# truemeat001/Simple-Raytracing-Render

Measured on AMD Instinct MI355X. Metric: Msamples/s (rays x bounces) + HBM GB/s vs roofline, Cornell+teapot 1024spp, higher is better.
Workload: dtype f32

## Files before the change

### include/srr_capi.h

```cpp
#ifndef SRR_CAPI_H
#define SRR_CAPI_H

#include <stddef.h>
#include <stdint.h>

#ifdef __cplusplus
extern "C" {
#endif

#define SRR_OK 0
#define SRR_EINVAL (-22)
#define SRR_ENOMEM (-12)
#define SRR_ENODEV (-19)
#define SRR_ENOTSUP (-95)
#define SRR_EIO (-5)

typedef struct srr_scene srr_scene;
typedef struct srr_renderer srr_renderer;

const char* srr_last_error(void);
const char* srr_version(void);

srr_scene* srr_scene_create(void);
void srr_scene_destroy(srr_scene* s);
int srr_scene_from_text(const char* text, srr_scene** out);
int srr_scene_text_handle(const srr_scene* s, int text_id);
int srr_scene_set_lcg(srr_scene* s, uint64_t state);
#define SRR_DIGEST_PARTS 21
int srr_scene_digest(const srr_scene* s, uint64_t* out, uint64_t* parts);
uint64_t srr_scene_get_lcg(const srr_scene* s);
double srr_scene_drand48(srr_scene* s);

int srr_constant_texture(srr_scene* s, float r, float g, float b);
int srr_image_texture(srr_scene* s, const unsigned char* rgb, int nx, int ny);
int srr_image_texture_file(srr_scene* s, const char* path);
int srr_image_texture_gen(srr_scene* s, int nx, int ny, uint32_t seed, int kind);
int srr_checker_texture(srr_scene* s, int even_tex, int odd_tex);
int srr_noise_texture(srr_scene* s, float scale);

int srr_lambertian(srr_scene* s, int albedo_tex);
int srr_orennayar(srr_scene* s, int albedo_tex, float sigma_deg);
int srr_beckmann(srr_scene* s, int albedo_tex, float roughx, float roughy);
int srr_metal(srr_scene* s, float r, float g, float b, float fuzz);
int srr_dielectric(srr_scene* s, float ref_idx);
int srr_diffuse_light(srr_scene* s, int emit_tex);
int srr_isotropic(srr_scene* s, int albedo_tex);

int srr_sphere(srr_scene* s, const float center[3], float radius, int mat);
int srr_moving_sphere(srr_scene* s, const float c0[3], const float c1[3], float t0, float t1, float radius,
                      int mat);
int srr_xy_rect(srr_scene* s, float x0, float x1, float y0, float y1, float k, int mat);
int srr_xz_rect(srr_scene* s, float x0, float x1, float z0, float z1, float k, int mat);
int srr_yz_rect(srr_scene* s, float y0, float y1, float z0, float z1, float k, int mat);
int srr_box(srr_scene* s, const float p0[3], const float p1[3], int mat);
int srr_triangle(srr_scene* s, const float p[9], int mat, const float* uv9, const float* n9);
int srr_flip_normals(srr_scene* s, int child);
int srr_translate(srr_scene* s, int child, const float offset[3]);
int srr_rotate_y(srr_scene* s, int child, float angle_deg);
int srr_rotate_x(srr_scene* s, int child, float angle_deg);
int srr_constant_medium(srr_scene* s, int boundary, float density, int tex);
int srr_hitable_list(srr_scene* s, const int* children, int n);
int srr_bvh_node(srr_scene* s, const int* children, int n, float time0, float time1);
// ... 110 lines not shown
```

### simple-raytracing-render_amd/csrc/capi.cpp

```cpp
#include <hip/hip_runtime.h>

#include <algorithm>
#include <chrono>
#include <cstdint>
#include <cstdio>
#include <cstring>
#include <map>
#include <memory>
#include <string>
#include <vector>

#include "../../include/srr_capi.h"
#include "imageio.h"
#include "meshio.h"
#include "../../include/srr/merl.h"
#include "multi.h"
#include "renderer.h"

using namespace srr;

struct srr_scene {
  Scene s;
};

// ... 74 lines not shown
  auto vec = [&blob](const auto& v) { blob(v.data(), v.size() * sizeof(v[0])); };
  vec(f.objs);
  blob(&f.n_world, sizeof f.n_world);
  vec(f.xforms);
  vec(f.spheres);
  vec(f.rects);
  vec(f.stris);
  vec(f.meshes);
  vec(f.nodes);
  vec(f.node4);
  vec(f.tri_pos);
  vec(f.tri_shade);
  vec(f.media);
  {
    std::vector<uint8_t> b;
    auto put = [&b](const void* p, size_t n) { b.insert(b.end(), (const uint8_t*)p, (const uint8_t*)p + n); };
    put(f.obvhs.data(), f.obvhs.size() * sizeof(DObvh));
    put(f.sgroups.data(), f.sgroups.size() * sizeof(DSGroup));
    put(f.sg_items.data(), f.sg_items.size() * sizeof(DSGItem));
    vec(b);
  }
  vec(f.obvh_children);
  vec(f.mats);
  vec(f.texs);
  vec(f.images);
  vec(f.perlin_ranvec);
  vec(f.perlin_perm);
  vec(f.lights);
  blob(&f.cam, sizeof f.cam);
  *out = h;
  return 0;
}

int srr_scene_set_lcg(srr_scene* s, uint64_t state) {
  if (!s) return fail(SRR_EINVAL, "null scene");
  s->s.lcg = state & 0xFFFFFFFFFFFFULL;
  return 0;
}
uint64_t srr_scene_get_lcg(const srr_scene* s) { return s ? s->s.lcg : 0; }
double srr_scene_drand48(srr_scene* s) { return s ? s->s.drand48() : 0.0; }

#define SCN(s) \
  if (!(s)) return fail(SRR_EINVAL, "null scene");
#define TEXOK(s, t) \
  if (!(s)->s.valid_tex(t)) return fail(SRR_EINVAL, "bad texture handle " + std::to_string(t));
#define MATOK(s, m) \
  if (!(s)->s.valid_mat(m)) return fail(SRR_EINVAL, "bad material handle " + std::to_string(m));
#define OBJOK(s, o) \
  if (!(s)->s.valid_obj(o)) return fail(SRR_EINVAL, "bad hitable handle " + std::to_string(o));

int srr_constant_texture(srr_scene* s, float r, float g, float b) {
  SCN(s);
  HTex t;
  t.kind = TEX_CONST;
  t.c[0] = r; t.c[1] = g; t.c[2] = b;
  return s->s.add_tex(std::move(t));
}
int srr_image_texture(srr_scene* s, const unsigned char* rgb, int nx, int ny) {
  SCN(s);
  if (!rgb || nx <= 0 || ny <= 0) return fail(SRR_EINVAL, "bad image");
  HTex t;
  t.kind = TEX_IMAGE;
  t.nx = nx;
  t.ny = ny;
  t.px.assign(rgb, rgb + (size_t)nx * ny * 3);
  return s->s.add_tex(std::move(t));
// ... 765 lines not shown
```

### simple-raytracing-render_amd/csrc/device_scene.h

```cpp
#pragma once
#include <cstdint>

namespace srr {

enum ObjKind : int32_t {
  OBJ_SPHERE = 0,
  OBJ_MSPHERE = 1,
  OBJ_RECT = 2,
  OBJ_TRI = 3,
  OBJ_MESH = 4,
  OBJ_MEDIUM = 5,
  OBJ_OBVH = 6,
  OBJ_SGROUP = 7,
};

enum XformKind : int32_t { XF_FLIP = 0, XF_TRANSLATE = 1, XF_ROTY = 2, XF_ROTX = 3 };

struct DXform {
  int32_t kind;
  float a, b, c;
};

constexpr int32_t kXfFlipBit = 1 << 30;
constexpr int32_t kXfCountMask = 0xFFFF;
// ... 2 lines not shown
  int32_t kind;
  int32_t xf_begin, xf_count;
  int32_t idx;
};

struct DSphere {
  float c0[3], c1[3];
  float t0, t1, r;
  int32_t mat;
};

struct DRect {
  int32_t kax, a0, a1, mat;
  float lo0, hi0, lo1, hi1, k;
  float pad[3];
};

struct TriShade {
  float n[9];
  float uv[6];
  int32_t mat;
};

constexpr int kNode4qWords = 16;

struct DMesh {
  int32_t node_off;
  int32_t tri_off;
  int32_t n_nodes, n_tris;
  int32_t node4_off;
  int32_t n_node4;
};

struct DObvh {
  int32_t node_off, n_nodes;
  int32_t child_off, n_children;
};

struct DObvhChild {
  int32_t obj_begin, obj_count;
};

constexpr int kSGroupMinRun = 8;

struct DSGroup {
  int32_t node_off, n_nodes;
  int32_t item_off, n_items;
};

struct DSGItem {
  DSphere s;
  int32_t pos;
  int32_t moving;
  int32_t obj;
  int32_t pad;
};

struct DMedium {
  int32_t bnd_begin, bnd_count;
  float density;
  int32_t phase_mat;
};

enum MatKind : int32_t {
  MAT_LAMBERTIAN = 0,
  MAT_ORENNAYAR = 1,
  MAT_BECKMANN = 2,
  MAT_METAL = 3,
  MAT_DIELECTRIC = 4,
  MAT_DIFFUSE_LIGHT = 5,
  MAT_ISOTROPIC = 6,
  MAT_COUNT = 7,
};

struct DMat {
  int32_t kind;
  int32_t tex;
  float p[4];
};

enum TexKind : int32_t { TEX_CONST = 0, TEX_IMAGE = 1, TEX_CHECKER = 2, TEX_NOISE = 3 };

struct DTex {
  int32_t kind;
  int32_t nx, ny;
  int32_t even, odd;
  int64_t off;
  float c[3];
};

enum LightKind : int32_t { LIGHT_NONE = 0, LIGHT_XZRECT = 1, LIGHT_SPHERE = 2, LIGHT_TRI = 3 };

struct DLight {
  int32_t kind;
// ... 15 lines not shown
```

### simple-raytracing-render_amd/csrc/kernels.h

```cpp
#pragma once
#include <hip/hip_runtime.h>

#include <cstdint>

#include "device_scene.h"

namespace srr {

struct SceneView {
  const DObj* objs;
  int n_world;
  int has_media;
  const DXform* xforms;
  const DSphere* spheres;
  const DRect* rects;
  const DStandaloneTri* stris;
  const DMesh* meshes;
  const float4* nodes;
  const float4* node4;
  int node4_lds;
  int node4_total;
  const float4* node4q;
  int node4_lds_q;
  int use_q;
  int quad_trace;
  int quad_max;
  int mesh_obj;
  const float4* tri_pos;
  const float4* tri_edge;
  const TriShade* tri_shade;
  const DMedium* media;
  const DObvh* obvhs;
  const DObvhChild* obvh_children;
  const DSGroup* sgroups;
  const DSGItem* sg_items;
  const DMat* mats;
  const DTex* texs;
  const uint8_t* images;
  const float* perlin_ranvec;
  const int32_t* perlin_perm;
  const DLight* lights;
  int n_lights;
  float light_weight;
  const DCamera* cam;
  const uint4* world_blob;
  int world_words;
  int world_off[10];
};

struct PathState {
  float4* ray_o;
  float4* ray_d;
  uint64_t* lcg;
  uint64_t* pcg;
  int32_t* depth;
  uint64_t* spec;
  int4* hit_w;
  float4* hit_p;
  float4* hit_n;
  float4* rec_a;
  float* sample;
  float* raw;
  uint8_t* rays;
};

struct BatchInfo {
  int32_t* active;
  int32_t* count;
  int act0;
  int slot0;
  const int32_t* pixels;
  const double* sobol;
  int p0;
  int n_paths;
  int s0, spp_batch;
  int s_base;
  int nx, ny;
  uint64_t base_seed;
};

// ... 97 lines not shown
```

### simple-raytracing-render_amd/csrc/kernels.hip

```cpp
#include <hip/hip_runtime.h>

#include <cfloat>
#include <algorithm>
#include <cstdint>
#include <cstdlib>
#include <cstring>

#include "device_scene.h"
#include "devmath.h"
#include "kernels.h"
#include "../../include/srr/merl.h"

namespace srr {
namespace dev {

SRR_D V3 sphere_center(const DSphere& s, float tm, bool moving) {
  V3 c0 = v3(s.c0[0], s.c0[1], s.c0[2]);
  if (!moving) return c0;
  V3 c1 = v3(s.c1[0], s.c1[1], s.c1[2]);
  return c0 + ((tm - s.t0) / (s.t1 - s.t0)) * (c1 - c0);
}

SRR_D bool sphere_hit(const DSphere& s, bool moving, const Ray& r, float tmin, float tmax, float& t) {
  V3 oc = r.o - sphere_center(s, r.tm, moving);
  float a = dot(r.d, r.d);
  float b = dot(oc, r.d);
  float c = dot(oc, oc) - s.r * s.r;
  float disc = b * b - a * c;
  if (disc > 0) {
    float sq = rsqrt_exact(disc);
    float temp = (-b - sq) / a;
    if (temp < tmax && temp > tmin) { t = temp; return true; }
    temp = (-b + sq) / a;
    if (temp < tmax && temp > tmin) { t = temp; return true; }
  }
  return false;
}

template <int KAX>
SRR_D bool rect_hit_t(const DRect& q, const Ray& r, float tmin, float tmax, float& t) {
  constexpr int A0 = KAX == 0 ? 1 : 0, A1 = KAX == 2 ? 1 : 2;
  const float tt = (q.k - r.o[KAX]) / r.d[KAX];
  if (tt < tmin || tt > tmax) return false;
  const float x = r.o[A0] + tt * r.d[A0];
  const float y = r.o[A1] + tt * r.d[A1];
  if (x < q.lo0 || x > q.hi0 || y < q.lo1 || y > q.hi1) return false;
  t = tt;
  return true;
}

#ifndef SRR_RECTAX
#define SRR_RECTAX 1
#endif
SRR_D bool rect_hit(const DRect& q, const Ray& r, float tmin, float tmax, float& t, float& u, float& v) {
#ifdef SRR_EXP_FASTRECT
  float tt = (q.k - r.o[q.kax]) * __builtin_amdgcn_rcpf(r.d[q.kax]);
#else
  float tt = (q.k - r.o[q.kax]) / r.d[q.kax];
#endif
  if (tt < tmin || tt > tmax) return false;
  float x = r.o[q.a0] + tt * r.d[q.a0];
  float y = r.o[q.a1] + tt * r.d[q.a1];
  if (x < q.lo0 || x > q.hi0 || y < q.lo1 || y > q.hi1) return false;
  u = (x - q.lo0) / (q.hi0 - q.lo0);
  v = (y - q.lo1) / (q.hi1 - q.lo1);
  t = tt;
  return true;
}

SRR_D bool tri_hit(V3 p0, V3 p1, V3 p2, bool front, V3 o, V3 dir, float& t, float& u, float& v) {
  V3 e1, e2;
  if (front) { e1 = p1 - p0; e2 = p2 - p0; }
  else { e1 = p0 - p1; e2 = p2 - p1; }
// ... 1149 lines not shown
      for (int i = first; i < first + count; ++i) {
        const DSGItem it = S.sg_items[i];
        const V3 oc = r.o - sphere_center(it.s, r.tm, it.moving != 0);
        const float a = dot(r.d, r.d);
        const float b = dot(oc, r.d);
        const float c = dot(oc, oc) - it.s.r * it.s.r;
        const float disc = b * b - a * c;
        if (!(disc > 0)) continue;
        const float sq = rsqrt_exact(disc);
        const float t1 = (-b - sq) / a;
        float v;
        if (t1 > tmin) v = t1;
        else {
          const float t2 = (-b + sq) / a;
          if (!(t2 > tmin)) continue;
          v = t2;
        }
        if (!(v < tmax)) continue;
        if (!found || v < best || (v == best && it.pos < best_pos)) {
          found = true;
          best = v;
          best_pos = it.pos;
          best_item = i;
        }
      }
    }
    node = (hit && leaf < 0) ? node + 1 : skip;
  }
  out_t = best;
  out_item = best_item;
  return found;
}

template <int TR, bool U = false>
SRR_D bool basic_hit(const SceneView& S, const DObj& ob, const Ray& lr, float tmin, float tmax, bool is_medium,
                     ObjHit& h, const TraceCtx& cx) {
  switch (ob.kind) {
    case OBJ_MESH: {
#ifdef SRR_EXP_NOMESH
      return false;
#endif
      MeshHit mh;
      const DMesh m = maybe_uni<U>(wload<TR>(S.meshes, ob.idx));
      bool hit;
      if (tr_mode(TR) == TR_BVH2) hit = mesh_hit<false>(S, m, lr, tmin, tmax, is_medium, mh, cx.ctr);
      else if (TR & TR_QUAD)
        hit = mesh_hit4_quad<tr_mode(TR) != TR_BVH4, tr_stride(TR)>(S, m, lr, tmin, tmax, is_medium, mh, cx);
      else if (TR & TR_Q)
        hit = mesh_hit4<tr_mode(TR) != TR_BVH4, false, true, tr_stride(TR)>(S, m, lr, tmin, tmax, is_medium, mh, cx);
      else
        hit = mesh_hit4<tr_mode(TR) != TR_BVH4, tr_mode(TR) == TR_BVH4_TIMED, false, tr_stride(TR), (TR & TR_SUSP) != 0>(
            S, m, lr, tmin, tmax, is_medium, mh, cx);
      if (!hit) return false;
      h.t = mh.t;
      h.prim = mh.tri;
      return true;
    }
    case OBJ_OBVH:
      return obvh_hit<TR>(S, S.obvhs[ob.idx], lr, tmin, tmax, is_medium, h.t, h.prim);
    case OBJ_SGROUP:
      return sgroup_hit<TR>(S, S.sgroups[ob.idx], lr, tmin, tmax, h.t, h.prim);
    case OBJ_MEDIUM:
      return false;
    default:
      return prim_hit<TR, U>(S, ob, lr, tmin, tmax, is_medium, h.t);
  }
}

template <int TR>
SRR_D bool list_hit(const SceneView& S, int b, int n, const Ray& r, float tmin, float tmax, float& t,
                    const TraceCtx& cx) {
  bool any = false;
  float closest = tmax;
  for (int k = 0; k < n; ++k) {
    const DObj ob = maybe_uni<SRR_UNIFORM != 0>(wload<TR>(S.objs, b + k));
    const Ray lr = chain_in<TR, SRR_UNIFORM != 0>(S, ob, r);
    float th = 0;
    bool hit;
    if (ob.kind == OBJ_MESH) {
      MeshHit mh;
      hit = mesh_hit<false>(S, wload<TR>(S.meshes, ob.idx), lr, tmin, closest, true, mh, nullptr);
      th = mh.t;
    } else if (ob.kind == OBJ_OBVH) {
      int po;
      hit = obvh_hit<TR>(S, S.obvhs[ob.idx], lr, tmin, closest, true, th, po);
    } else if (ob.kind == OBJ_MEDIUM) {
      hit = false;
    } else {
      hit = prim_hit<TR, SRR_UNIFORM != 0>(S, ob, lr, tmin, closest, true, th);
    }
    if (hit) {
      any = true;
      closest = th;
      t = th;
    }
  }
  return any;
}
// ... 44 lines not shown
    if (MEDIA && ob.kind == OBJ_MEDIUM) {
      hit = medium_hit<TR>(S, maybe_uni<SRR_UNIFORM != 0>(wload<TR>(S.media, ob.idx)), lr, tmin, closest, rng, h.t, cx);
      h.prim = -1;
    } else {
      hit = basic_hit<TR, SRR_UNIFORM != 0>(S, ob, lr, tmin, closest, false, h, cx);
    }
    if (hit) {
      closest = h.t;
      w.obj = k;
      w.prim = h.prim;
      w.t = h.t;
    }
  }
}

template <bool MEDIA, int TR>
SRR_D WorldHit world_hit(const SceneView& S, const Ray& r, Rng& rng, const TraceCtx& cx) {
  WorldHit w{-1, -1, 0};
  float closest = FLT_MAX;
  const float tmin = 0.001f;
  constexpr bool SUSP = (TR & TR_SUSP) != 0;
  const bool skip = MEDIA || S.mesh_obj < 0;
  int k_res = -1;
  if constexpr (SUSP) {
    if (skip && cx.resume) {
      const float4 v = *walk_save(cx, 2);
      k_res = __float_as_int(v.x);
      closest = v.y;
      w.obj = __float_as_int(v.z);
      w.prim = __float_as_int(v.w);
      w.t = closest;
    }
  }
  for (int k = 0; k < S.n_world; ++k) {
    const DObj ob = maybe_uni<SRR_UNIFORM != 0>(wload<TR>(S.objs, k));
    if constexpr (SUSP) {
      if (skip && (cx.susp || k < k_res)) continue;
      cx.obj_k = k;
    }
    Ray lr = chain_in<TR, SRR_UNIFORM != 0>(S, ob, r);
    ObjHit h;
    bool hit;
    if (MEDIA && ob.kind == OBJ_MEDIUM) {
      hit = medium_hit<TR>(S, maybe_uni<SRR_UNIFORM != 0>(wload<TR>(S.media, ob.idx)), lr, tmin, closest, rng, h.t, cx);
      h.prim = -1;
    } else {
      hit = basic_hit<TR, SRR_UNIFORM != 0>(S, ob, lr, tmin, closest, false, h, cx);
    }
    if (SUSP && skip && cx.susp) {
      *walk_save(cx, 2) = make_float4(__int_as_float(k), closest, __int_as_float(w.obj), __int_as_float(w.prim));
      continue;
    }
    if (hit) {
      closest = h.t;
      w.obj = k;
      w.prim = h.prim;
      w.t = h.t;
    }
  }
  return w;
}

struct HitRec {
  V3 p, n;
  float u, v;
  int mat;
};

#if SRR_XFAX
template <int KAX>
SRR_D void rect_rec(const DRect& q, const Ray& r, HitRec& h) {
  constexpr int A0 = KAX == 0 ? 1 : 0, A1 = KAX == 2 ? 1 : 2;
  const float tt = (q.k - r.o[KAX]) / r.d[KAX];
  const float x = r.o[A0] + tt * r.d[A0];
  const float y = r.o[A1] + tt * r.d[A1];
  h.u = (x - q.lo0) / (q.hi0 - q.lo0);
  h.v = (y - q.lo1) / (q.hi1 - q.lo1);
  h.n = v3(0.f);
  h.n.set(KAX, 1.f);
}
#endif

SRR_D void sphere_uv(V3 p, float& u, float& v) {
  float phi = ratan2(p.z, p.x);
  float theta = rasin(p.y);
  u = 1 - (phi + kPi) / (2 * kPi);
  v = (theta + kPi / 2) / kPi;
}

template <int TR = 0>
SRR_D void prim_record(const SceneView& S, const DObj& ob, const Ray& lr, float t, int prim, HitRec& h) {
  switch (ob.kind) {
    case OBJ_SPHERE:
    case OBJ_MSPHERE: {
      const DSphere& s = S.spheres[ob.idx];
      V3 c = sphere_center(s, lr.tm, ob.kind == OBJ_MSPHERE);
      h.p = lr.at(t);
      if (ob.kind == OBJ_SPHERE) sphere_uv((h.p - c) / s.r, h.u, h.v);
      h.n = (h.p - c) / s.r;
      h.mat = s.mat;
      break;
    }
    case OBJ_RECT: {
      const DRect& q = S.rects[ob.idx];
#if SRR_XFAX
      switch (q.kax) {
        case 0: rect_rec<0>(q, lr, h); break;
        case 1: rect_rec<1>(q, lr, h); break;
        default: rect_rec<2>(q, lr, h); break;
      }
#else
      float tt;
      rect_hit(q, lr, -FLT_MAX, FLT_MAX, tt, h.u, h.v);
      h.n = v3(0.f);
      h.n.set(q.kax, 1.f);
#endif
      h.p = lr.at(t);
      h.mat = q.mat;
      break;
    }
    case OBJ_TRI:
    case OBJ_MESH: {
      V3 p0, p1, p2;
      TriShade shv;
      if (ob.kind == OBJ_TRI) {
        DStandaloneTri T;
        if constexpr ((TR & TR_WL) != 0) {
          static_assert(sizeof(DStandaloneTri) == 25 * 4, "DStandaloneTri: 25 words");
          const __attribute__((address_space(3))) float* q =
              (const __attribute__((address_space(3))) float*)(S.stris + ob.idx);
          float* t = (float*)&T;
#pragma unroll
          for (int k = 0; k < 25; ++k) t[k] = q[k];
        } else {
          T = S.stris[ob.idx];
// ... 7 lines not shown
        float4 a = tp[0], b = tp[1], c = tp[2];
        p0 = v3(a.x, a.y, a.z);
        p1 = v3(b.x, b.y, b.z);
        p2 = v3(c.x, c.y, c.z);
        shv = S.tri_shade[prim];
      }
      const TriShade* sh = &shv;
      V3 dir = lr.d / length(lr.d);
      float tt, u, v;
      tri_hit(p0, p1, p2, true, lr.o, dir, tt, u, v);
      float a0 = 1 - u - v;
      float uvx = a0 * sh->uv[0] + u * sh->uv[2] + v * sh->uv[4];
      float uvy = a0 * sh->uv[1] + u * sh->uv[3] + v * sh->uv[5];
      h.u = uvx;
      h.v = uvy;
      V3 n0 = v3(sh->n[0], sh->n[1], sh->n[2]), n1 = v3(sh->n[3], sh->n[4], sh->n[5]),
         n2 = v3(sh->n[6], sh->n[7], sh->n[8]);
      h.n = unit_vector(a0 * n0 + u * n1 + v * n2);
      h.p = a0 * p0 + u * p1 + v * p2;
      h.mat = sh->mat;
      break;
    }
    case OBJ_MEDIUM: {
      h.p = lr.at(t);
      h.n = v3(1, 0, 0);
      h.mat = S.media[ob.idx].phase_mat;
      break;
    }
  }
}

template <int TR = 0>
SRR_D HitRec world_record(const SceneView& S, const Ray& r, const WorldHit& w) {
  const DObj& ob = S.objs[w.obj];
  Ray lr = chain_in<TR>(S, ob, r);
  HitRec h;
  h.u = 0;
  h.v = 0;
  if (ob.kind == OBJ_OBVH || ob.kind == OBJ_SGROUP) {
    const DObj& in = S.objs[ob.kind == OBJ_SGROUP ? S.sg_items[w.prim].obj : w.prim];
    prim_record<TR>(S, in, chain_in<TR>(S, in, lr), w.t, -1, h);
    chain_out(S, in, h.p, h.n);
  } else {
    prim_record<TR>(S, ob, lr, w.t, w.prim, h);
  }
  chain_out(S, ob, h.p, h.n);
  return h;
}

enum Family : int { FAM_TERM = 0, FAM_DIFF = 1, FAM_BECK = 2, FAM_SPEC = 3 };

SRR_D int family_of(int mat, int kind, int depth, int max_depth) {
  if (mat < 0 || kind == MAT_DIFFUSE_LIGHT || depth >= max_depth) return FAM_TERM;
  if (kind == MAT_LAMBERTIAN || kind == MAT_ORENNAYAR) return FAM_DIFF;
  if (kind == MAT_BECKMANN) return FAM_BECK;
  return FAM_SPEC;
}

SRR_D int hit_material(const SceneView& S, const WorldHit& w) {
  DObj ob = S.objs[w.obj];
  if (ob.kind == OBJ_OBVH) ob = S.objs[w.prim];
  else if (ob.kind == OBJ_SGROUP) ob = S.objs[S.sg_items[w.prim].obj];
  switch (ob.kind) {
    case OBJ_SPHERE:
    case OBJ_MSPHERE: return S.spheres[ob.idx].mat;
    case OBJ_RECT: return S.rects[ob.idx].mat;
    case OBJ_TRI: return S.stris[ob.idx].sh.mat;
    case OBJ_MESH: return S.tri_shade[w.prim].mat;
    case OBJ_MEDIUM: return S.media[ob.idx].phase_mat;
  }
  return -1;
}

SRR_D void store_hit(const SceneView& S, const PathState& P, int p, const WorldHit& w, int max_depth, int& fam) {
  if (w.obj < 0) {
// ... 1248 lines not shown
SRR_D const PathsArgs* paths_args() { return nullptr; }
#endif

template <bool MEDIA, bool ALLFAM, int MINB, bool TIMED = false, bool WL = true, bool QUAD = false, bool CQ = false,
          int BS = kPathsBlock, bool SP = false>
#ifdef SRR_NUM_VGPR
#define SRR_PATHS_VGPR_ATTR __attribute__((amdgpu_num_vgpr(SRR_NUM_VGPR)))
#else
#define SRR_PATHS_VGPR_ATTR
#endif
__global__ void __launch_bounds__(BS, MINB) SRR_PATHS_VGPR_ATTR k_paths(PathsArgs A) {
  static_assert(BS == kPathsBlock || BS == 1024, "block size");
  (void)A;
  uint64_t tp[8] = {0, 0, 0, 0, 0, 0, 0, 0};
  uint64_t tf[20] = {0, 0, 0, 0, 0, 0, 0, 0, 0, 0, 0, 0, 0, 0, 0, 0, 0, 0, 0, 0};
  uint64_t it = 0;
  constexpr int TR = TR_BVH4_PRUNE | (WL ? TR_WL : 0) | (QUAD ? TR_QUAD : 0) | (CQ ? TR_Q : 0) | (BS == 1024 ? TR_BIG : 0) |
                     ((SP && !QUAD && !CQ) ? TR_SUSP : 0);
  __shared__ uint4 s_world[WL ? kWorldLdsBytes / 16 : 1];
  const auto view = [&]() {
    SceneView S = paths_args()->S;
    if constexpr (WL) {
      const char* b = (const char*)s_world;
      S.objs = (const DObj*)(b + S.world_off[0]);
      S.xforms = (const DXform*)(b + S.world_off[1]);
      S.spheres = (const DSphere*)(b + S.world_off[2]);
      S.rects = (const DRect*)(b + S.world_off[3]);
      S.stris = (const DStandaloneTri*)(b + S.world_off[4]);
      S.meshes = (const DMesh*)(b + S.world_off[5]);
      S.media = (const DMedium*)(b + S.world_off[6]);
      S.mats = (const DMat*)(b + S.world_off[7]);
      S.texs = (const DTex*)(b + S.world_off[8]);
      S.lights = (const DLight*)(b + S.world_off[9]);
    }
    return S;
  };
  const auto work = []() { return PathWork(paths_args()->W); };
  __shared__ int s_node[kStack * BS];
  __shared__ float s_t[kStack * BS];
  constexpr bool RING = SRR_RAYRING && !QUAD;
  constexpr int kNodesLds = BS == 1024 ? kPathsLdsNodesBig : ((WL && RING) ? kPathsLdsNodesSmall : kPathsLdsNodes);
  __shared__ float4 s_n4[kNodesLds * 8];
  __shared__ float s_ring[RING ? kRingWords * BS : 1];
  const lds_ptr<float> ringw = to_lds(s_ring + (RING ? (threadIdx.x & ~63u) : 0));
  uint32_t ring_base = 0;
  const uint32_t n_paths = (uint32_t)paths_args()->W.n_paths;
  const uint64_t t_start = paths_args()->W.wave_times ? __builtin_amdgcn_s_memrealtime() : 0;
  {
    const SceneView S0 = paths_args()->S;
    if constexpr (WL)
      for (int i = threadIdx.x; i < S0.world_words; i += blockDim.x) s_world[i] = S0.world_blob[i];
    const int n_lds_nodes = CQ ? min(S0.node4_total, 2 * kNodesLds) : min(S0.node4_total, kNodesLds);
    if (CQ)
      for (int i = threadIdx.x; i < n_lds_nodes * 4; i += blockDim.x) s_n4[i] = S0.node4q[i];
    else
      for (int i = threadIdx.x; i < n_lds_nodes * 8; i += blockDim.x) s_n4[i] = S0.node4[i];
  }
  __syncthreads();
  const int slot = blockIdx.x * blockDim.x + threadIdx.x;
  const auto rec_at = [&](const PathWork& W, int k) -> float4* {
    int s = slot;
    asm volatile("" : "+v"(s));
    return W.rec + ((size_t)k * W.lanes + s);
  };
  int g = -1;
  uint32_t pool = 0, pool_end = 0;
// ... 1189 lines not shown
```

### simple-raytracing-render_amd/csrc/renderer.cpp

```cpp
#include "renderer.h"

#include "multi.h"

#include <algorithm>
#include <chrono>
#include <cstdlib>
#include <cstring>
#include <memory>
#include <thread>
#include <cstdio>

namespace srr {

constexpr int kCtrWords = 40;
constexpr int kVisitWords = 3 + 2 * 64;

#define RCHK(x)                                                        \
  do {                                                                 \
    hipError_t e_ = (x);                                               \
    if (e_ != hipSuccess) {                                            \
      err = std::string(#x) + ": " + hipGetErrorString(e_);            \
      return SRR_EIO;                                                  \
    }                                                                  \
  } while (0)
// ... 40 lines not shown
  float* n4q;
  RCHK(upload(&n4q, F.node4q, K));
  RCHK(upload(&tp, F.tri_pos, K));
  float* tedge;
  {
    const size_t nt = F.tri_pos.size() / 16;
    std::vector<float> pr(32 * nt, 0.f);
    for (size_t i = 0; i < nt; ++i)
      for (int j = 0; j < 2; ++j) {
        const float* q = &F.tri_pos[16 * std::min(i + j, nt - 1)];
        float* o = &pr[32 * i + 9 * j];
        for (int c = 0; c < 3; ++c) {
          o[c] = q[c];
          o[3 + c] = q[4 + c] - q[c];
          o[6 + c] = q[8 + c] - q[c];
        }
      }
    RCHK(upload(&tedge, pr, K));
  }
  RCHK(upload(&ts, F.tri_shade, K));
  RCHK(upload(&md, F.media, K));
  RCHK(upload(&ob, F.obvhs, K));
  RCHK(upload(&oc, F.obvh_children, K));
  RCHK(upload(&sg, F.sgroups, K));
  RCHK(upload(&sgi, F.sg_items, K));
  RCHK(upload(&mt, F.mats, K));
  RCHK(upload(&tx, F.texs, K));
  RCHK(upload(&im, F.images, K));
  RCHK(upload(&pr, F.perlin_ranvec, K));
  RCHK(upload(&pp, F.perlin_perm, K));
  RCHK(upload(&li, F.lights, K));
  RCHK(upload(&cm, cam, K));
  std::vector<uint8_t> blob;
  int off[10];
  auto put = [&](int k, const void* data, size_t bytes) {
    off[k] = (int)blob.size();
    blob.insert(blob.end(), (const uint8_t*)data, (const uint8_t*)data + bytes);
    blob.resize((blob.size() + 15) & ~(size_t)15, 0);
  };
  put(0, F.objs.data(), F.objs.size() * sizeof(DObj));
  put(1, F.xforms.data(), F.xforms.size() * sizeof(DXform));
  put(2, F.spheres.data(), F.spheres.size() * sizeof(DSphere));
  put(3, F.rects.data(), F.rects.size() * sizeof(DRect));
  put(4, F.stris.data(), F.stris.size() * sizeof(DStandaloneTri));
  put(5, F.meshes.data(), F.meshes.size() * sizeof(DMesh));
  put(6, F.media.data(), F.media.size() * sizeof(DMedium));
  put(7, F.mats.data(), F.mats.size() * sizeof(DMat));
  put(8, F.texs.data(), F.texs.size() * sizeof(DTex));
  put(9, F.lights.data(), F.lights.size() * sizeof(DLight));
  uint8_t* wb;
  RCHK(upload(&wb, blob, K));
  SceneView& V = r->view;
  V.world_blob = (const uint4*)wb;
  V.world_words = (int)(blob.size() / 16);
  for (int k = 0; k < 10; ++k) V.world_off[k] = off[k];
  V.objs = objs;
  V.n_world = F.n_world;
  V.has_media = F.media.empty() ? 0 : 1;
  V.xforms = xf;
  V.spheres = sph;
  V.rects = rct;
  V.stris = st;
  V.meshes = me;
  V.nodes = (const float4*)nodes;
  V.node4 = (const float4*)n4;
  V.node4_lds = (int)std::min<size_t>(kPathsLdsNodes, F.node4.size() / 32);
  V.node4_total = (int)(F.node4.size() / 32);
  V.node4q = F.node4q_ok && !F.node4q.empty() ? (const float4*)n4q : nullptr;
  V.node4_lds_q = (int)std::min<size_t>(2 * kPathsLdsNodes, F.node4q.size() / kNode4qWords);
  {
    const char* e = getenv("SRR_CBVH");
    V.use_q = V.node4q && e && atoi(e) != 0;
  }
  {
    const char* e = getenv("SRR_QUAD");
    V.quad_trace = e ? (atoi(e) != 0) : false;
    const char* q = getenv("SRR_QUAD_MAX");
    V.quad_max = q ? atoi(q) : 32;
  }
  {
    int n_mesh = 0;
    V.mesh_obj = -1;
    for (int k = 0; k < F.n_world; ++k)
      if (F.objs[k].kind == OBJ_MESH) {
        ++n_mesh;
        V.mesh_obj = k;
      }
    if (n_mesh != 1) V.mesh_obj = -1;
// ... 1057 lines not shown
```

### simple-raytracing-render_amd/csrc/scene.cpp

```cpp
#include "scene.h"

#include <algorithm>
#include <array>
#include <cfloat>
#include <cmath>
#include <cstdio>
#include <cstdlib>
#include <cstring>
#include <fstream>
#include <functional>
#include <iterator>
#include <map>
#include <sstream>

namespace srr {

static const double kPi = 3.14159265358979323846;
static const uint64_t kPostPerlinSeed = 24561125610955ULL;

#include "../../include/srr/teapot_data.inc"

Scene::Scene() : lcg(kPostPerlinSeed) {}

double Scene::drand48() {
// ... 1397 lines not shown
  if (!fl.walk(S.world, {}, fl.world, false)) return -95;
  std::vector<DObj> grouped_objs;
  const std::vector<DObj> world = group_sphere_runs(S, F, fl.world, grouped_objs);
  F.n_world = (int)world.size();
  F.objs = world;
  for (DObj d : fl.bound) F.objs.push_back(d);
  for (DMedium& m : F.media) m.bnd_begin += F.n_world;
  const int inner_base = (int)F.objs.size();
  for (DObj d : fl.inner) F.objs.push_back(d);
  for (DObvhChild& c : F.obvh_children) c.obj_begin += inner_base;
  const int grouped_base = (int)F.objs.size();
  for (DObj d : grouped_objs) F.objs.push_back(d);
  for (DSGItem& it : F.sg_items) it.obj += grouped_base;
  for (int k : S.obj[S.lights].kids) {
    if (S.obj[k].kind == H_LIST) {
      err = "nested hitable_list inside the light list is not supported";
      return -95;
    }
    F.lights.push_back(fl.light(k));
  }
  compact_materials(F);
  perlin_tables(F.perlin_ranvec, F.perlin_perm);
  const HCamera& c = S.cam;
  std::memcpy(F.cam.origin, c.origin, 12);
  std::memcpy(F.cam.llc, c.llc, 12);
  std::memcpy(F.cam.horizontal, c.horizontal, 12);
  std::memcpy(F.cam.vertical, c.vertical, 12);
  std::memcpy(F.cam.u, c.u, 12);
  std::memcpy(F.cam.v, c.v, 12);
  F.cam.time0 = c.time0;
  F.cam.time1 = c.time1;
  F.cam.lens_radius = c.lens_radius;
  return 0;
}

namespace {
struct Tok {
  std::vector<std::string> t;
  int line;
  float f(size_t i) const { return std::strtof(t.at(i).c_str(), nullptr); }
  long long i(size_t k) const { return std::strtoll(t.at(k).c_str(), nullptr, 10); }
  unsigned long long u(size_t k) const { return std::strtoull(t.at(k).c_str(), nullptr, 10); }
  void v3(size_t k, float* o) const { o[0] = f(k); o[1] = f(k + 1); o[2] = f(k + 2); }
};
}

int scene_from_text(const std::string& text, Scene& S, std::string& err) {
  std::istringstream is(text);
  std::string line;
  int ln = 0;
  bool header = false;
  std::map<long long, int> T, M, O;
  std::map<long long, std::pair<int, int>> G;
  auto need = [&](std::map<long long, int>& mp, long long id, const char* what) -> int {
    if (id == -1 && std::string(what) == "mat") return -1;
    auto it = mp.find(id);
    if (it == mp.end()) throw std::runtime_error(std::string("undefined ") + what + " " + std::to_string(id));
    return it->second;
  };
  try {
    while (std::getline(is, line)) {
      ++ln;
      size_t h = line.find('#');
      if (h != std::string::npos) line.resize(h);
      Tok c;
      c.line = ln;
// ... 118 lines not shown
```

### simple-raytracing-render_amd/csrc/scene.h

```cpp
#pragma once
#include <cstdint>
#include <string>
#include <vector>

#include "device_scene.h"

namespace srr {

enum HKind : int32_t {
  H_SPHERE, H_MSPHERE, H_XY, H_XZ, H_YZ, H_BOX, H_TRI, H_FLIP, H_TRANSLATE, H_ROTY, H_ROTX, H_MEDIUM, H_LIST, H_BVH
};

struct Box3 {
  float mn[3], mx[3];
};

struct HTex {
  TexKind kind;
  float c[3] = {0, 0, 0};
  int nx = 0, ny = 0;
  std::vector<uint8_t> px;
  int even = -1, odd = -1;
};

// ... 81 lines not shown

int scene_from_text(const std::string& text, Scene& s, std::string& err);

struct Flat {
  std::vector<DObj> objs;
  int n_world = 0;
  std::vector<DXform> xforms;
  std::vector<DSphere> spheres;
  std::vector<DRect> rects;
  std::vector<DStandaloneTri> stris;
  std::vector<DMesh> meshes;
  std::vector<float> nodes;
  std::vector<float> node4;
  std::vector<float> node4q;
  bool node4q_ok = true;
  std::vector<float> tri_pos;
  std::vector<TriShade> tri_shade;
  std::vector<DMedium> media;
  std::vector<DObvh> obvhs;
  std::vector<DObvhChild> obvh_children;
  std::vector<DSGroup> sgroups;
  std::vector<DSGItem> sg_items;
  std::vector<DMat> mats;
  std::vector<DTex> texs;
  std::vector<uint8_t> images;
  std::vector<float> perlin_ranvec;
  std::vector<int32_t> perlin_perm;
  std::vector<DLight> lights;
  DCamera cam{};
};

int flatten(const Scene& s, Flat& f, std::string& err);

void teapot_triangles(float scale, int divs, std::vector<float>& p9);

uint64_t path_seed(uint32_t x, uint32_t y, uint32_t s, uint64_t base);

void sobol2(unsigned n, double* out);

std::vector<uint8_t> gen_image(int w, int h, uint32_t seed, int kind);

}
```

Baseline: 9066.

## Pack top-level world objects into fixed 64-byte records with inlined primitive data

Builds a per-world-object record (DWRec) that inlines the object header with its rect, sphere, mesh or medium payload and material kind. The trace loop then loads it as one 64-byte record through the constant address space instead of chasing an index into separate tables. Hit-record reconstruction also reads from these records. The aim is fewer dependent scalar loads per object per ray, at the cost of a larger per-object load and duplicated scene data. It also adds a C API to export the flattened tables.

```diff
diff --git a/include/srr_capi.h b/include/srr_capi.h
--- a/include/srr_capi.h
+++ b/include/srr_capi.h
@@ -28,6 +28,18 @@
 int srr_scene_set_lcg(srr_scene* s, uint64_t state);
 #define SRR_DIGEST_PARTS 21
 int srr_scene_digest(const srr_scene* s, uint64_t* out, uint64_t* parts);
+enum {
+  SRR_TABLE_OBJECTS = 0,
+  SRR_TABLE_N_WORLD = 1,
+  SRR_TABLE_SPHERES = 2,
+  SRR_TABLE_RECTS = 3,
+  SRR_TABLE_MESHES = 4,
+  SRR_TABLE_MEDIA = 5,
+  SRR_TABLE_MATERIALS = 6,
+  SRR_TABLE_WORLD_RECORDS = 7
+};
+int srr_scene_tables(const srr_scene* s, int n_tables, const int* tables, void* const* outs, const int64_t* caps,
+                     int64_t* sizes);
 uint64_t srr_scene_get_lcg(const srr_scene* s);
 double srr_scene_drand48(srr_scene* s);
 
diff --git a/simple-raytracing-render_amd/csrc/capi.cpp b/simple-raytracing-render_amd/csrc/capi.cpp
--- a/simple-raytracing-render_amd/csrc/capi.cpp
+++ b/simple-raytracing-render_amd/csrc/capi.cpp
@@ -130,6 +130,35 @@
   return 0;
 }
 
+int srr_scene_tables(const srr_scene* s, int n_tables, const int* tables, void* const* outs, const int64_t* caps,
+                     int64_t* sizes) {
+  if (!s || !tables || !sizes || n_tables < 0) return fail(SRR_EINVAL, "null argument");
+  Flat f;
+  std::string err;
+  const int rc = flatten(s->s, f, err);
+  if (rc < 0) return fail(rc, err);
+  const std::vector<DWRec> wrecs = world_records(f);
+  for (int i = 0; i < n_tables; ++i) {
+    const void* p = nullptr;
+    size_t n = 0;
+    auto vec = [&](const auto& v) { p = v.data(), n = v.size() * sizeof(v[0]); };
+    switch (tables[i]) {
+      case SRR_TABLE_OBJECTS: vec(f.objs); break;
+      case SRR_TABLE_N_WORLD: p = &f.n_world, n = sizeof f.n_world; break;
+      case SRR_TABLE_SPHERES: vec(f.spheres); break;
+      case SRR_TABLE_RECTS: vec(f.rects); break;
+      case SRR_TABLE_MESHES: vec(f.meshes); break;
+      case SRR_TABLE_MEDIA: vec(f.media); break;
+      case SRR_TABLE_MATERIALS: vec(f.mats); break;
+      case SRR_TABLE_WORLD_RECORDS: vec(wrecs); break;
+      default: return fail(SRR_EINVAL, "unknown table");
+    }
+    if (outs && caps && outs[i] && caps[i] >= (int64_t)n && n) std::memcpy(outs[i], p, n);
+    sizes[i] = (int64_t)n;
+  }
+  return 0;
+}
+
 int srr_scene_set_lcg(srr_scene* s, uint64_t state) {
   if (!s) return fail(SRR_EINVAL, "null scene");
   s->s.lcg = state & 0xFFFFFFFFFFFFULL;
diff --git a/simple-raytracing-render_amd/csrc/device_scene.h b/simple-raytracing-render_amd/csrc/device_scene.h
--- a/simple-raytracing-render_amd/csrc/device_scene.h
+++ b/simple-raytracing-render_amd/csrc/device_scene.h
@@ -58,6 +58,30 @@
   int32_t n_node4;
 };
 
+struct DMedium {
+  int32_t bnd_begin, bnd_count;
+  float density;
+  int32_t phase_mat;
+};
+
+struct DRectCore {
+  int32_t kax, a0, a1, mat;
+  float lo0, hi0, lo1, hi1, k;
+};
+struct DWRec {
+  DObj ob;
+  int32_t mat;
+  int32_t mat_kind;
+  union {
+    DRectCore rect;
+    DSphere sphere;
+    DMesh mesh;
+    DMedium medium;
+    uint32_t w[10];
+  };
+};
+static_assert(sizeof(DWRec) == 64, "DWRec: 16 words");
+
 struct DObvh {
   int32_t node_off, n_nodes;
   int32_t child_off, n_children;
@@ -80,12 +104,6 @@
   int32_t moving;
   int32_t obj;
   int32_t pad;
-};
-
-struct DMedium {
-  int32_t bnd_begin, bnd_count;
-  float density;
-  int32_t phase_mat;
 };
 
 enum MatKind : int32_t {
diff --git a/simple-raytracing-render_amd/csrc/kernels.h b/simple-raytracing-render_amd/csrc/kernels.h
--- a/simple-raytracing-render_amd/csrc/kernels.h
+++ b/simple-raytracing-render_amd/csrc/kernels.h
@@ -45,7 +45,9 @@
   const DCamera* cam;
   const uint4* world_blob;
   int world_words;
-  int world_off[10];
+  int world_off[11];
+  const DWRec* wrecs;
+  const DWRec* wrecs_hit;
 };
 
 struct PathState {
diff --git a/simple-raytracing-render_amd/csrc/kernels.hip b/simple-raytracing-render_amd/csrc/kernels.hip
--- a/simple-raytracing-render_amd/csrc/kernels.hip
+++ b/simple-raytracing-render_amd/csrc/kernels.hip
@@ -37,8 +37,8 @@
   return false;
 }
 
-template <int KAX>
-SRR_D bool rect_hit_t(const DRect& q, const Ray& r, float tmin, float tmax, float& t) {
+template <int KAX, class Q>
+SRR_D bool rect_hit_t(const Q& q, const Ray& r, float tmin, float tmax, float& t) {
   constexpr int A0 = KAX == 0 ? 1 : 0, A1 = KAX == 2 ? 1 : 2;
   const float tt = (q.k - r.o[KAX]) / r.d[KAX];
   if (tt < tmin || tt > tmax) return false;
@@ -1254,30 +1254,34 @@
   return found;
 }
 
+template <int TR>
+SRR_D bool mesh_obj_hit(const SceneView& S, const DMesh& m, const Ray& lr, float tmin, float tmax, bool is_medium,
+                        ObjHit& h, const TraceCtx& cx) {
+#ifdef SRR_EXP_NOMESH
+  return false;
+#endif
+  MeshHit mh;
+  bool hit;
+  if (tr_mode(TR) == TR_BVH2) hit = mesh_hit<false>(S, m, lr, tmin, tmax, is_medium, mh, cx.ctr);
+  else if (TR & TR_QUAD)
+    hit = mesh_hit4_quad<tr_mode(TR) != TR_BVH4, tr_stride(TR)>(S, m, lr, tmin, tmax, is_medium, mh, cx);
+  else if (TR & TR_Q)
+    hit = mesh_hit4<tr_mode(TR) != TR_BVH4, false, true, tr_stride(TR)>(S, m, lr, tmin, tmax, is_medium, mh, cx);
+  else
+    hit = mesh_hit4<tr_mode(TR) != TR_BVH4, tr_mode(TR) == TR_BVH4_TIMED, false, tr_stride(TR), (TR & TR_SUSP) != 0>(
+        S, m, lr, tmin, tmax, is_medium, mh, cx);
+  if (!hit) return false;
+  h.t = mh.t;
+  h.prim = mh.tri;
+  return true;
+}
+
 template <int TR, bool U = false>
 SRR_D bool basic_hit(const SceneView& S, const DObj& ob, const Ray& lr, float tmin, float tmax, bool is_medium,
                      ObjHit& h, const TraceCtx& cx) {
   switch (ob.kind) {
-    case OBJ_MESH: {
-#ifdef SRR_EXP_NOMESH
-      return false;
-#endif
-      MeshHit mh;
-      const DMesh m = maybe_uni<U>(wload<TR>(S.meshes, ob.idx));
-      bool hit;
-      if (tr_mode(TR) == TR_BVH2) hit = mesh_hit<false>(S, m, lr, tmin, tmax, is_medium, mh, cx.ctr);
-      else if (TR & TR_QUAD)
-        hit = mesh_hit4_quad<tr_mode(TR) != TR_BVH4, tr_stride(TR)>(S, m, lr, tmin, tmax, is_medium, mh, cx);
-      else if (TR & TR_Q)
-        hit = mesh_hit4<tr_mode(TR) != TR_BVH4, false, true, tr_stride(TR)>(S, m, lr, tmin, tmax, is_medium, mh, cx);
-      else
-        hit = mesh_hit4<tr_mode(TR) != TR_BVH4, tr_mode(TR) == TR_BVH4_TIMED, false, tr_stride(TR), (TR & TR_SUSP) != 0>(
-            S, m, lr, tmin, tmax, is_medium, mh, cx);
-      if (!hit) return false;
-      h.t = mh.t;
-      h.prim = mh.tri;
-      return true;
-    }
+    case OBJ_MESH:
+      return mesh_obj_hit<TR>(S, maybe_uni<U>(wload<TR>(S.meshes, ob.idx)), lr, tmin, tmax, is_medium, h, cx);
     case OBJ_OBVH:
       return obvh_hit<TR>(S, S.obvhs[ob.idx], lr, tmin, tmax, is_medium, h.t, h.prim);
     case OBJ_SGROUP:
@@ -1286,6 +1290,41 @@
       return false;
     default:
       return prim_hit<TR, U>(S, ob, lr, tmin, tmax, is_medium, h.t);
+  }
+}
+
+#ifndef SRR_WRECS
+#define SRR_WRECS 1
+#endif
+SRR_D DWRec wrec_load(const SceneView& S, int k) {
+#if defined(__HIP_DEVICE_COMPILE__)
+  return ((const __attribute__((address_space(4))) DWRec*)(uintptr_t)S.wrecs)[k];
+#else
+  return S.wrecs[k];
+#endif
+}
+
+template <int TR>
+SRR_D bool rec_hit(const SceneView& S, const DWRec& rc, const Ray& lr, float tmin, float tmax, ObjHit& h,
+                   const TraceCtx& cx) {
+  switch (rc.ob.kind) {
+    case OBJ_RECT:
+#if SRR_RECTAX
+      switch (rc.rect.kax) {
+        case 0: return rect_hit_t<0>(rc.rect, lr, tmin, tmax, h.t);
+        case 1: return rect_hit_t<1>(rc.rect, lr, tmin, tmax, h.t);
+        default: return rect_hit_t<2>(rc.rect, lr, tmin, tmax, h.t);
+      }
+#else
+      return prim_hit<TR, SRR_UNIFORM != 0>(S, rc.ob, lr, tmin, tmax, false, h.t);
+#endif
+    case OBJ_SPHERE:
+    case OBJ_MSPHERE:
+      return sphere_hit(rc.sphere, rc.ob.kind == OBJ_MSPHERE, lr, tmin, tmax, h.t);
+    case OBJ_MESH:
+      return mesh_obj_hit<TR>(S, rc.mesh, lr, tmin, tmax, false, h, cx);
+    default:
+      return basic_hit<TR, SRR_UNIFORM != 0>(S, rc.ob, lr, tmin, tmax, false, h, cx);
   }
 }
 
@@ -1396,8 +1435,15 @@
       w.t = closest;
     }
   }
+#if SRR_WRECS
+#endif
   for (int k = 0; k < S.n_world; ++k) {
+#if SRR_WRECS
+    const DWRec rc = maybe_uni<SRR_UNIFORM != 0>(wrec_load(S, k));
+    const DObj ob = rc.ob;
+#else
     const DObj ob = maybe_uni<SRR_UNIFORM != 0>(wload<TR>(S.objs, k));
+#endif
     if constexpr (SUSP) {
       if (skip && (cx.susp || k < k_res)) continue;
       cx.obj_k = k;
@@ -1405,12 +1451,21 @@
     Ray lr = chain_in<TR, SRR_UNIFORM != 0>(S, ob, r);
     ObjHit h;
     bool hit;
+#if SRR_WRECS
+    if (MEDIA && ob.kind == OBJ_MEDIUM) {
+      hit = medium_hit<TR>(S, rc.medium, lr, tmin, closest, rng, h.t, cx);
+      h.prim = -1;
+    } else {
+      hit = rec_hit<TR>(S, rc, lr, tmin, closest, h, cx);
+    }
+#else
     if (MEDIA && ob.kind == OBJ_MEDIUM) {
       hit = medium_hit<TR>(S, maybe_uni<SRR_UNIFORM != 0>(wload<TR>(S.media, ob.idx)), lr, tmin, closest, rng, h.t, cx);
       h.prim = -1;
     } else {
       hit = basic_hit<TR, SRR_UNIFORM != 0>(S, ob, lr, tmin, closest, false, h, cx);
     }
+#endif
     if (SUSP && skip && cx.susp) {
       *walk_save(cx, 2) = make_float4(__int_as_float(k), closest, __int_as_float(w.obj), __int_as_float(w.prim));
       continue;
@@ -1432,10 +1487,9 @@
 };
 
 #if SRR_XFAX
-template <int KAX>
-SRR_D void rect_rec(const DRect& q, const Ray& r, HitRec& h) {
+template <int KAX, class Q>
+SRR_D void rect_rec_t(const Q& q, const Ray& r, float tt, HitRec& h) {
   constexpr int A0 = KAX == 0 ? 1 : 0, A1 = KAX == 2 ? 1 : 2;
-  const float tt = (q.k - r.o[KAX]) / r.d[KAX];
   const float x = r.o[A0] + tt * r.d[A0];
   const float y = r.o[A1] + tt * r.d[A1];
   h.u = (x - q.lo0) / (q.hi0 - q.lo0);
@@ -1443,6 +1497,10 @@
   h.n = v3(0.f);
   h.n.set(KAX, 1.f);
 }
+template <int KAX>
+SRR_D void rect_rec(const DRect& q, const Ray& r, HitRec& h) {
+  rect_rec_t<KAX>(q, r, (q.k - r.o[KAX]) / r.d[KAX], h);
+}
 #endif
 
 SRR_D void sphere_uv(V3 p, float& u, float& v) {
@@ -1452,19 +1510,21 @@
   v = (theta + kPi / 2) / kPi;
 }
 
+SRR_D void sphere_record(const DSphere& s, int kind, const Ray& lr, float t, HitRec& h) {
+  V3 c = sphere_center(s, lr.tm, kind == OBJ_MSPHERE);
+  h.p = lr.at(t);
+  if (kind == OBJ_SPHERE) sphere_uv((h.p - c) / s.r, h.u, h.v);
+  h.n = (h.p - c) / s.r;
+  h.mat = s.mat;
+}
+
 template <int TR = 0>
 SRR_D void prim_record(const SceneView& S, const DObj& ob, const Ray& lr, float t, int prim, HitRec& h) {
   switch (ob.kind) {
     case OBJ_SPHERE:
-    case OBJ_MSPHERE: {
-      const DSphere& s = S.spheres[ob.idx];
-      V3 c = sphere_center(s, lr.tm, ob.kind == OBJ_MSPHERE);
-      h.p = lr.at(t);
-      if (ob.kind == OBJ_SPHERE) sphere_uv((h.p - c) / s.r, h.u, h.v);
-      h.n = (h.p - c) / s.r;
-      h.mat = s.mat;
+    case OBJ_MSPHERE:
+      sphere_record(S.spheres[ob.idx], ob.kind, lr, t, h);
       break;
-    }
     case OBJ_RECT: {
       const DRect& q = S.rects[ob.idx];
 #if SRR_XFAX
@@ -1538,7 +1598,12 @@
 
 template <int TR = 0>
 SRR_D HitRec world_record(const SceneView& S, const Ray& r, const WorldHit& w) {
+#if SRR_WRECS
+  const DWRec& rc = S.wrecs_hit[w.obj];
+  const DObj ob = rc.ob;
+#else
   const DObj& ob = S.objs[w.obj];
+#endif
   Ray lr = chain_in<TR>(S, ob, r);
   HitRec h;
   h.u = 0;
@@ -1547,6 +1612,20 @@
     const DObj& in = S.objs[ob.kind == OBJ_SGROUP ? S.sg_items[w.prim].obj : w.prim];
     prim_record<TR>(S, in, chain_in<TR>(S, in, lr), w.t, -1, h);
     chain_out(S, in, h.p, h.n);
+#if SRR_WRECS && SRR_XFAX && SRR_RECTAX
+  } else if (ob.kind == OBJ_RECT) {
+    switch (rc.rect.kax) {
+      case 0: rect_rec_t<0>(rc.rect, lr, w.t, h); break;
+      case 1: rect_rec_t<1>(rc.rect, lr, w.t, h); break;
+      default: rect_rec_t<2>(rc.rect, lr, w.t, h); break;
+    }
+    h.p = lr.at(w.t);
+    h.mat = rc.rect.mat;
+#endif
+#if SRR_WRECS
+  } else if (ob.kind == OBJ_SPHERE || ob.kind == OBJ_MSPHERE) {
+    sphere_record(rc.sphere, ob.kind, lr, w.t, h);
+#endif
   } else {
     prim_record<TR>(S, ob, lr, w.t, w.prim, h);
   }
@@ -2861,6 +2940,7 @@
       S.mats = (const DMat*)(b + S.world_off[7]);
       S.texs = (const DTex*)(b + S.world_off[8]);
       S.lights = (const DLight*)(b + S.world_off[9]);
+      S.wrecs_hit = (const DWRec*)(b + S.world_off[10]);
     }
     return S;
   };
diff --git a/simple-raytracing-render_amd/csrc/renderer.cpp b/simple-raytracing-render_amd/csrc/renderer.cpp
--- a/simple-raytracing-render_amd/csrc/renderer.cpp
+++ b/simple-raytracing-render_amd/csrc/renderer.cpp
@@ -96,7 +96,7 @@
   RCHK(upload(&li, F.lights, K));
   RCHK(upload(&cm, cam, K));
   std::vector<uint8_t> blob;
-  int off[10];
+  int off[11];
   auto put = [&](int k, const void* data, size_t bytes) {
     off[k] = (int)blob.size();
     blob.insert(blob.end(), (const uint8_t*)data, (const uint8_t*)data + bytes);
@@ -112,12 +112,18 @@
   put(7, F.mats.data(), F.mats.size() * sizeof(DMat));
   put(8, F.texs.data(), F.texs.size() * sizeof(DTex));
   put(9, F.lights.data(), F.lights.size() * sizeof(DLight));
+  const std::vector<DWRec> wrecs = world_records(F);
+  DWRec* wr;
+  RCHK(upload(&wr, wrecs, K));
+  put(10, wrecs.data(), wrecs.size() * sizeof(DWRec));
   uint8_t* wb;
   RCHK(upload(&wb, blob, K));
   SceneView& V = r->view;
+  V.wrecs = wr;
+  V.wrecs_hit = wr;
   V.world_blob = (const uint4*)wb;
   V.world_words = (int)(blob.size() / 16);
-  for (int k = 0; k < 10; ++k) V.world_off[k] = off[k];
+  for (int k = 0; k < 11; ++k) V.world_off[k] = off[k];
   V.objs = objs;
   V.n_world = F.n_world;
   V.has_media = F.media.empty() ? 0 : 1;
diff --git a/simple-raytracing-render_amd/csrc/scene.cpp b/simple-raytracing-render_amd/csrc/scene.cpp
--- a/simple-raytracing-render_amd/csrc/scene.cpp
+++ b/simple-raytracing-render_amd/csrc/scene.cpp
@@ -1453,6 +1453,39 @@
   F.cam.time1 = c.time1;
   F.cam.lens_radius = c.lens_radius;
   return 0;
+}
+
+std::vector<DWRec> world_records(const Flat& F) {
+  std::vector<DWRec> out((size_t)F.n_world + 1);
+  std::memset(out.data(), 0, out.size() * sizeof(DWRec));
+  for (int k = 0; k < F.n_world; ++k) {
+    DWRec& r = out[k];
+    r.ob = F.objs[k];
+    r.mat = -1;
+    switch (r.ob.kind) {
+      case OBJ_RECT:
+        static_assert(offsetof(DRect, k) == offsetof(DRectCore, k), "DRectCore: DRect's leading words");
+        std::memcpy(&r.rect, &F.rects[r.ob.idx], sizeof(DRectCore));
+        r.mat = r.rect.mat;
+        break;
+      case OBJ_SPHERE:
+      case OBJ_MSPHERE:
+        std::memcpy(&r.sphere, &F.spheres[r.ob.idx], sizeof(DSphere));
+        r.mat = r.sphere.mat;
+        break;
+      case OBJ_MESH:
+        std::memcpy(&r.mesh, &F.meshes[r.ob.idx], sizeof(DMesh));
+        break;
+      case OBJ_MEDIUM:
+        std::memcpy(&r.medium, &F.media[r.ob.idx], sizeof(DMedium));
+        r.mat = r.medium.phase_mat;
+        break;
+      default:
+        break;
+    }
+    r.mat_kind = r.mat >= 0 && r.mat < (int)F.mats.size() ? F.mats[r.mat].kind : -1;
+  }
+  return out;
 }
 
 namespace {
diff --git a/simple-raytracing-render_amd/csrc/scene.h b/simple-raytracing-render_amd/csrc/scene.h
--- a/simple-raytracing-render_amd/csrc/scene.h
+++ b/simple-raytracing-render_amd/csrc/scene.h
@@ -137,6 +137,8 @@
 
 int flatten(const Scene& s, Flat& f, std::string& err);
 
+std::vector<DWRec> world_records(const Flat& f);
+
 void teapot_triangles(float scale, int divs, std::vector<float>& p9);
 
 uint64_t path_seed(uint32_t x, uint32_t y, uint32_t s, uint64_t base);
```

New measurement: 9088, median of 6. No clear change (+0.2%).
